# bcgsc/abyss

Measured on AMD Instinct MI355X. Metric: Mk-mers/s inserted+extended (abyss-bloom-dbg, k=64); unitig bit-exact, higher is better.
Workload: dtype u64

## Files before the change

### abyss_amd/_lib.py

```python
from __future__ import annotations

import ctypes as C
import os

from . import build

ABG_OK = 0
ABG_EINVAL, ABG_ENODEV, ABG_ENOMEM, ABG_EINTERNAL, ABG_EAGAIN = -1, -2, -3, -4, -5


class Params(C.Structure):
    _fields_ = [
        ("k", C.c_uint32), ("num_hashes", C.c_uint32), ("min_cov", C.c_uint32), ("trim", C.c_uint32),
        ("bloom_bytes", C.c_uint64), ("counters", C.c_uint64), ("spaced_seed", C.c_char_p),
        ("device", C.c_int32), ("verbose", C.c_int32), ("insert_batch_kmers", C.c_uint64),
        ("claim_log2", C.c_uint32), ("walk_slots", C.c_uint32), ("wtab_log2", C.c_uint32),
        ("cascade_levels", C.c_uint32), ("slice_filter", C.c_uint32), ("reserved_", C.c_uint32 * 5),
    ]


class Counters(C.Structure):
    _fields_ = [(n, C.c_uint64) for n in
                ("solid_reads", "visited_reads", "reads_processed", "bases_assembled", "next_contig_id")]


class Contig(C.Structure):
    _fields_ = [
        ("contig_id", C.c_uint64), ("read_index", C.c_uint64), ("seq", C.c_char_p),
        ("length", C.c_uint32), ("coverage", C.c_uint32), ("redundant", C.c_int32),
        ("left_ext", C.c_uint32), ("right_ext", C.c_uint32), ("left_code", C.c_int32),
        ("right_code", C.c_int32), ("seed_pos", C.c_uint32),
    ]


class Stats(C.Structure):
    _fields_ = [(n, C.c_uint64) for n in
                ("insert_rounds", "walk_rounds", "candidates", "walked", "rewalked", "commit_breaks",
                 "commit_rounds", "generated", "bulk_calls", "bulk_steps", "lin_steps", "guide_slots", "chain_steps", "batch_cuts", "overflows", "memo_hits", "memo_adds", "tiled_ops", "tiled_pending", "tile_overflows", "cls_covered_reads", "archive_bases", "cls_decided_reads", "counter_bytes_held",
                 "commit_rounds_incremental", "commit_dirty_records", "commit_first_chunk_decided")]


CONTIG_CB = C.CFUNCTYPE(None, C.c_void_p, C.POINTER(Contig))
TEXT_CB = C.CFUNCTYPE(None, C.c_void_p, C.POINTER(C.c_char), C.c_uint64)

_lib = None

STAGE_PREFIXES = [("abg_overlap", True), ("abg_rr", True), ("abg_kn", True), ("abg_fm", True), ("abg_de", True), ("abg_ov", True),
                  ("abg_sg", True), ("abg_mc", True), ("abg_pb", False), ("abg_mp", False)]


def symbols():
    return [
        "abg_params_init", "abg_create", "abg_destroy", "abg_last_error", "abg_reset", "abg_filter_size",
        "abg_load_seqs", "abg_load_seqs_v", "abg_keep_reads", "abg_assemble_kept", "abg_load_packed", "abg_counting_stats", "abg_counters_export",
        "abg_counters_import", "abg_visited_export", "abg_visited_import", "abg_assemble_seqs", "abg_assemble_seqs_v",
        "abg_assemble_packed", "abg_cascade_export", "abg_get_counters", "abg_set_counters", "abg_hash_seq",
        "abg_contains_seq",
        "abg_attach_comm", "abg_share_reads", "abg_rccl_unique_id", "abg_rccl_comm_create", "abg_rccl_comm_destroy",
        "abg_dev_copy", "abg_dev_alloc", "abg_dev_free", "abg_output_graph_seqs",
        "abg_profile_enable", "abg_profile_reset", "abg_profile_get", "abg_get_stats",
        "abg_overlap_create", "abg_overlap_destroy", "abg_overlap_last_error", "abg_overlap_join", "abg_overlap_edges",
        "abg_overlap_profile", "abg_overlap_profile_get",
        "abg_rr_create", "abg_rr_destroy", "abg_rr_last_error", "abg_rr_bytes", "abg_rr_clear", "abg_rr_insert_seqs",
        "abg_rr_contains_seqs", "abg_rr_popcount", "abg_rr_export", "abg_rr_sync", "abg_rr_profile", "abg_rr_profile_get",
        "abg_kn_create", "abg_kn_destroy", "abg_kn_last_error", "abg_kn_import", "abg_kn_export", "abg_kn_insert_seqs",
        "abg_kn_contains_seqs", "abg_kn_popcount", "abg_kn_hash_seq", "abg_kn_sync", "abg_kn_profile", "abg_kn_profile_get",
        "abg_fm_create", "abg_fm_destroy", "abg_fm_last_error", "abg_fm_build", "abg_fm_size", "abg_fm_export", "abg_fm_map_seqs",
        "abg_fm_sync", "abg_fm_tune", "abg_fm_profile", "abg_fm_profile_get",
        "abg_de_create", "abg_de_destroy", "abg_de_last_error", "abg_de_set_pmf", "abg_de_scan", "abg_de_estimate", "abg_de_tune",
        "abg_de_profile", "abg_de_profile_get",
        "abg_ov_create", "abg_ov_destroy", "abg_ov_last_error", "abg_ov_set_contigs", "abg_ov_find", "abg_ov_profile",
        "abg_ov_profile_get",
        "abg_sg_create", "abg_sg_destroy", "abg_sg_last_error", "abg_sg_set_graph", "abg_sg_search", "abg_sg_tune", "abg_sg_profile",
        "abg_sg_profile_get",
        "abg_mc_create", "abg_mc_destroy", "abg_mc_last_error", "abg_mc_set_contigs", "abg_mc_merge", "abg_mc_tune", "abg_mc_profile",
        "abg_mc_profile_get",
        "abg_pb_create", "abg_pb_destroy", "abg_pb_last_error", "abg_pb_tune", "abg_pb_align", "abg_pb_align_chain", "abg_pb_profile_get",
        "abg_pb_profile_reset",
        "abg_mp_create", "abg_mp_destroy", "abg_mp_last_error", "abg_mp_tune", "abg_mp_align", "abg_mp_profile_get", "abg_mp_profile_reset",
    ]


def load(path: str | None = None):
    global _lib
    if _lib is not None:
        return _lib
    if path is None:
        path = os.environ.get("ABG_LIB") or build.LIB
        if not os.path.exists(path):
            build.build_lib()
    lib = C.CDLL(path)
    vp, u64p, u8p = C.c_void_p, C.POINTER(C.c_uint64), C.c_void_p
# ... 103 lines not shown
```

### abyss_amd/csrc/abg_engine.h

```cpp
#pragma once
#include "abg_walk.h"

#include <algorithm>
#include <chrono>
#include <cstdio>
#include <cstdlib>
#include <cstring>
#include <functional>
#include <future>
#include <string>
#include <type_traits>
#include <vector>

namespace abg {

struct Failure { int code; std::string msg; };
constexpr int FAIL_INVAL = -1, FAIL_NOMEM = -3, FAIL_INTERNAL = -4;
[[noreturn]] inline void fail_now(int code, const std::string& msg) { throw Failure{ code, msg }; }
inline std::string strf(const char* fmt, unsigned long long a = 0, unsigned long long b = 0)
{
	char buf[256];
	snprintf(buf, sizeof buf, fmt, a, b);
	return buf;
}

struct Config {
	uint32_t k = 0, nh = 4, kc = 2, trim = 0;
	uint64_t counters = 0;
	uint32_t cascade_levels = 0;
	std::string spaced_seed;
	uint64_t insert_batch_kmers = 1ull << 24;
	uint32_t claim_log2 = 30;
	uint32_t drain_threshold = 1u << 12;
	uint64_t compact_threshold = 1u << 20;
	bool async_load = true;
	bool tiled_insert = true;
	bool benign_sharers = true;
	uint32_t cls_debug_skip = 0;
	bool cls_archive = true;
	uint32_t cls_archive_max_mb = 16384;
	bool sorted_overflow = true;
	bool cosettle = true;
	uint32_t cosettle_passes = 6;
	uint32_t cosettle_log2 = 24;
	uint32_t walk_slots = 4096;
	uint32_t tb_cap = 512;
	uint32_t buf_cap = 1u << 16;
	uint64_t pool_cap = 1ull << 28;
	uint32_t rec_cap = 1u << 22;
	uint32_t wtab_log2 = 26;
	uint32_t wtab_log2_max = 31;
	uint32_t cend_log2 = 20;
	uint64_t p2_first_batch = 65536;
	uint64_t p2_max_batch = 1ull << 22;
	uint32_t p2_growth = 2;
	uint32_t p2_crowded = 1u << 18;
	uint32_t p2_starved_growth = 2;
	uint32_t p2_starved = 6144;
	uint32_t slice_filter = 0;
	bool solid_plane = true;
	uint32_t classify_slots = 65536;
	uint32_t cls_both_max_mb = 1024;
	bool cls_both = true;
	bool prefetch_classify = true;
	uint32_t memo_log2 = 0;
	bool memo = true;
	uint32_t p2_max_candidates = 1u << 18;
	uint32_t t_tags = 1024;
	uint32_t commit_incremental = 1;
	uint32_t commit_dirty_max = 4096;
	uint32_t commit_dirty_log2 = 26;
	uint32_t guide_stride = 4;
	uint32_t guide_log2_max = 31;
	bool guide_seen = true;
	bool link_duplicates = true;
	bool par_commit = true;
	bool overlap_bins = true;
	bool overlap_purity = true;
	bool apply_mask = true;
	bool lead_implicit = true;
	uint32_t dist_hash_all_ranks = 2;
	uint32_t dist_route_min_ranks = 4;
	uint64_t keep_insert_scratch_bytes = 16ull << 30;
	uint64_t par_commit_max_bytes = 16ull << 30;
	int verbose = 0;
};

struct Counters {
	uint64_t solid_reads = 0, visited_reads = 0, reads_processed = 0, bases_assembled = 0,
	         contig_id = 0;
};

struct BaseCodes {
	uint8_t t[256];
	BaseCodes()
	{
		for (int i = 0; i < 256; i++) t[i] = 0xFF;
		t['A'] = t['a'] = 0; t['C'] = t['c'] = 1; t['G'] = t['g'] = 2; t['T'] = t['t'] = 3;
	}
};
template <class T>
struct NoInitAlloc : std::allocator<T> {
	template <class U> struct rebind { using other = NoInitAlloc<U>; };
	template <class U, class... A> void construct(U* p, A&&... a)
	{
		if constexpr (sizeof...(A) == 0) ::new ((void*)p) U; else ::new ((void*)p) U(std::forward<A>(a)...);
	}
};
struct HostBatch {
	std::vector<uint32_t, NoInitAlloc<uint32_t>> words;
	std::vector<uint64_t> woff{ 0 };
	std::vector<uint32_t> len;
	std::vector<uint64_t> koff{ 0 };
	void clear() { words.clear(); woff.assign(1, 0); len.clear(); koff.assign(1, 0); }
// ... 2618 lines not shown
						both_set(e.both32, pos);
						if (e.cnt8) { const unsigned c = e.cnt8[pos]; mn = c < mn ? c : mn; }
					}
					if (e.cnt8) cov += mn;
				}
				if (cov) atomic_add_u32(&rec.coverage, cov);
			}
		}
		if (lane == 0) { e.cnt[i] = nrec; e.cnt2[i] = nins; e.cnt3[i] = bases; }
	}
};
struct FPcCover {
	ParCommit e; uint8_t* kmin; uint32_t sum;
	ABG_HDN void operator()(uint64_t i, uint32_t lane, uint32_t nlanes) const
	{
		const uint32_t c = e.c_begin + (uint32_t)i;
		if (c >= e.brk || !e.active[i]) return;
		for (uint32_t ri = e.first_rec[c]; ri != REC_END; ri = e.recs[ri].next) {
			ContigRec& rec = e.recs[ri];
			if (!rec.ins) continue;
			const uint64_t* ch = e.kh + rec.seq_off;
			const uint32_t cnk = rec.len - e.p.k + 1;
			uint32_t cov = 0;
			for (uint32_t j = lane; j < cnk; j += nlanes) {
				if (sum) { cov += kmin[rec.seq_off + j]; continue; }
				const uint64_t h = ch[j];
				unsigned mn = 255;
				for (unsigned q = 0; q < e.p.nh; q++) {
					const uint64_t pos = pos_i(e.p, h, q);
					if (pos - e.own_lo < e.own_span) { const unsigned v = e.cnt8[pos]; mn = v < mn ? v : mn; }
				}
				kmin[rec.seq_off + j] = (uint8_t)mn;
			}
			if (sum && cov) atomic_add_u32(&rec.coverage, cov);
		}
	}
};
struct FPcWrite {
	ParCommit e; uint32_t* order; uint32_t order_base; uint64_t id_base;
	ABG_HD void operator()(uint64_t i, uint32_t) const
	{
		const uint32_t c = e.c_begin + (uint32_t)i;
		if (c >= e.brk || !e.active[i]) return;
		uint32_t o = order_base + e.cnt[i];
		uint64_t id = id_base + e.cnt2[i];
		for (uint32_t ri = e.first_rec[c]; ri != REC_END; ri = e.recs[ri].next) {
			ContigRec& rec = e.recs[ri];
			order[o++] = ri;
			if (rec.ins) rec.contig_id = id++;
		}
	}
};

template <class BE>
class Engine {
  public:
	Engine(BE& be, const Config& cfg) : be_(be), cfg_(cfg)
	{
		uint64_t rem = cfg_.counters % 8;
		m_ = rem ? cfg_.counters + 8 - rem : cfg_.counters;
		p_ = make_params(cfg_.k, cfg_.nh, cfg_.kc, cfg_.trim, m_);
		if (!cfg_.spaced_seed.empty()) {
			MaskTab* mt = new MaskTab;
			make_mask(cfg_.spaced_seed.c_str(), cfg_.k, *mt, p_);
			mask_d_ = (MaskTab*)be_.alloc(sizeof(MaskTab));
			be_.h2d(mask_d_, mt, sizeof(MaskTab));
			delete mt;
			p_.mask = mask_d_;
		}
		if (cfg_.cascade_levels) {
			casc_.levels = cfg_.cascade_levels;
			casc_.level_words = (m_ + 31) / 32;
			casc_.bits = (uint32_t*)be_.alloc(casc_.levels * casc_.level_words * 4);
			be_.memset(casc_.bits, 0, casc_.levels * casc_.level_words * 4);
			cnt_ = (uint8_t*)be_.alloc(8);
			vis_bytes_ = 8;
		} else {
			const uint64_t dev = be_.device_mem_bytes();
			cnt_deferred_ = cfg_.slice_filter == 1 || (cfg_.slice_filter == 0 && dev && (double)m_ * 1.3 > (double)dev * 0.9);
			if (!cnt_deferred_) {
				cnt_ = (uint8_t*)be_.alloc(m_ + 64 * (MAX_RANKS + 1));
				be_.memset(cnt_, 0, m_);
			}
			vis_bytes_ = (m_ / 8 + 4 + 3) & ~3ull;
		}
		vis_ = (uint8_t*)be_.alloc(vis_bytes_);
		be_.memset(vis_, 0, vis_bytes_);
		cstate_ = (CommitState*)be_.alloc(sizeof(CommitState));
		be_.memset(cstate_, 0, sizeof(CommitState));
		scal_ = (uint64_t*)be_.alloc(64);
	}
	~Engine()
	{
		if (BE::ITEM_GROUP_LOG2 == 0 && getenv("ABG_LEAD_COUNT"))
			fprintf(stderr, "lead_stores made=%llu skipped=%llu\n", (unsigned long long)stats_.lead_stores[0], (unsigned long long)stats_.lead_stores[1]);
		free_counters(); be_.free(vis_); if (both_) be_.free(both_); be_.free(cstate_); be_.free(scal_);
		free_archive();
		if (casc_.bits) be_.free(casc_.bits);
		if (mask_d_) be_.free(mask_d_);
		if (T_) be_.free(T_);
		if (Tk_) { be_.free(Tk_); be_.free(Tv_); }
		if (pcA_) be_.free(pcA_);
		if (la_pool_c_) be_.free(la_pool_c_);
		if (la_pool_c2_) be_.free(la_pool_c2_);
		if (guide_tab_) be_.free(guide_tab_);
		if (guide_seen_) be_.free(guide_seen_);
// ... 465 lines not shown
	}
	ContigArchive arc_{}; bool arc_valid_ = false;
	uint64_t loaded_ops_ = 0;
	uint64_t ovf_seen_[2] = { 0, 0 };
	uint8_t* plane_ = nullptr; bool plane_valid_ = false;
	Params p2_; const uint8_t* cnt2_ = nullptr;

	void build_guide(const Batch& b)
	{
		guide_.tab = nullptr; guide_.seen = nullptr; guide_slots_ = 0;
		if (!cfg_.guide_stride || p_.nh > 8 || !b.n) return;
		const uint64_t sampled = (b.n + cfg_.guide_stride - 1) / cfg_.guide_stride;
		uint64_t nwords = 0;
		be_.d2h(&nwords, b.woff + b.n, 8);
		const uint64_t bases = nwords * 16, minus = b.n * (uint64_t)(p_.k - 1);
		const uint64_t kmers = (bases > minus ? bases - minus : b.n) / std::min<uint32_t>(cfg_.guide_stride, 4u);
		uint32_t log2 = 16;
		while ((1ull << log2) < kmers && log2 < cfg_.guide_log2_max) log2++;
		if (!guide_tab_ || log2 != guide_log2_) {
			if (guide_tab_) be_.free(guide_tab_);
			guide_tab_ = (uint64_t*)be_.try_alloc(8ull << log2);
			guide_log2_ = log2;
			if (!guide_tab_) { if (cfg_.verbose) fprintf(stderr, "abyss_amd: no memory for the walkers' guide table, walking step by step\n"); return; }
		}
		be_.memset(guide_tab_, 0, 8ull << log2);
		guide_.mask = (1ull << log2) - 1; guide_.words = b.words; guide_.nwords = nwords;
		dispatch_nw([&](auto nw) {
			FGuideBuild<decltype(nw)::value> f{ p2_, b, cnt2_, guide_tab_, guide_.mask, cfg_.guide_stride, sampled };
			be_.launch_wave((sampled + GUIDE_READS_PER_ITEM - 1) / GUIDE_READS_PER_ITEM, f, "guide_build");
		});
		guide_.tab = guide_tab_;
		guide_slots_ = guide_.mask + 1;
		if (cfg_.guide_seen) {
			const uint64_t need = nwords * 16, total = be_.device_mem_bytes();
			if (guide_seen_ && guide_seen_bytes_ < need) { be_.free(guide_seen_); guide_seen_ = nullptr; }
			if (!guide_seen_ && (!total || need <= total / 24)) { guide_seen_ = (uint8_t*)be_.try_alloc(need); guide_seen_bytes_ = need; }
			if (guide_seen_) { be_.memset(guide_seen_, 0, need); guide_.seen = guide_seen_; }
		}
	}
	uint64_t next_batch_size() const
	{
		if (last_candidates_ > cfg_.p2_crowded) return std::max<uint64_t>(p2_batch_ / 2, 1024);
		if (last_candidates_ < cfg_.p2_starved) return std::min<uint64_t>(p2_batch_ * cfg_.p2_starved_growth, 8 * cfg_.p2_max_batch);
		return std::min<uint64_t>(p2_batch_ * cfg_.p2_growth, cfg_.p2_max_batch);
	}
	void clear_wstats()
	{
		be_.memset(wstats_, 0, WSTAT_N * 8);
	}
	struct Stats { uint64_t rounds = 0, walked = 0, rewalked = 0, candidates = 0, breaks = 0, insert_rounds = 0, commit_rounds = 0, generated = 0;
	               uint64_t bulk_calls = 0, bulk_steps = 0, lin_steps = 0, guide_slots = 0, chain_steps = 0, batch_cuts = 0, overflows = 0, memo_hits = 0, memo_adds = 0;
	               uint64_t tiled_ops = 0, tiled_pending = 0, tile_overflows = 0, cls_covered_reads = 0, archive_bases = 0, cls_decided_reads = 0;
	               uint64_t lead_stores[2] = { 0, 0 };
	               uint64_t commit_rounds_incremental = 0, commit_dirty_records = 0, commit_first_chunk_decided = 0; };
	Stats stats()
	{
		Stats s = stats_;
		if (wstats_) {
			uint64_t v[WSTAT_N];
			be_.d2h(v, wstats_, sizeof v);
			s.bulk_calls = v[WSTAT_BULK_CALLS]; s.bulk_steps = v[WSTAT_BULK_STEPS]; s.lin_steps = v[WSTAT_LIN_STEPS]; s.chain_steps = v[WSTAT_CHAIN_STEPS];
			s.memo_hits = v[WSTAT_MEMO_HITS]; s.memo_adds = v[WSTAT_MEMO_ADDS];
			s.cls_covered_reads = v[WSTAT_CLS_COVERED]; s.cls_decided_reads = v[WSTAT_CLS_DECIDED];
		}
		if (arc_.seq && arc_valid_) { uint64_t u = 0; be_.d2h(&u, arc_.used, 8); s.archive_bases = std::min(u, arc_.cap) - ARC_HEAD; }
		s.guide_slots = guide_slots_;
		return s;
	}

  private:
	BE& be_;
	Config cfg_;
	Params p_;
	uint64_t m_ = 0, vis_bytes_ = 0;
	uint8_t* cnt_ = nullptr;
	uint8_t* vis_ = nullptr;
	CommitState* cstate_ = nullptr;
	uint64_t* scal_ = nullptr;
	Cascade casc_{ nullptr, 0, 0 };
	MaskTab* mask_d_ = nullptr;
	std::chrono::steady_clock::time_point dbg_t0_;
	uint32_t* T_ = nullptr;
	uint32_t t_tag_ = 0;
	uint64_t* Tk_ = nullptr; uint32_t* Tv_ = nullptr; uint32_t Tlog2_ = 0;
	uint64_t T_entries_ = 0;
	uint32_t* pcA_ = nullptr; uint64_t pcA_bits_ = 0; uint32_t pcA_shift_ = 0;
	bool t_hashed() const { return t_force_hashed_ || m_ * 4ull > cfg_.par_commit_max_bytes; }
	bool t_force_hashed_ = false;
	bool use_par_commit()
	{
		if (!cfg_.par_commit || t_failed_) return false;
		if (t_hashed()) return true;
		if (!T_) {
			T_ = (uint32_t*)be_.try_alloc(m_ * 4ull);
			t_tag_ = 0;
			if (!T_ && sliced_) {
				t_force_hashed_ = true;
				if (cfg_.verbose) fprintf(stderr, "abyss_amd: no memory for a time stamp per filter bit, hashed stamps instead\n");
				return true;
			}
			if (!T_) { t_failed_ = true; if (cfg_.verbose) fprintf(stderr, "abyss_amd: no memory for the parallel commit's time stamps, using the ordered kernel\n"); return false; }
		}
		return true;
	}
	bool t_failed_ = false;
	Comm comm_;
	bool force_dist_ = false, comm_scaled_ = false;
	bool sliced_ = false, cnt_deferred_ = false; uint64_t win_total_ = 0, win_span_ = 0, win_lo_ = 0;
	bool cnt_loaded_ = false;
	uint64_t own_lo_ = 0, own_span_ = 0, own_chunk_ = 0;
	uint8_t* tred_ = nullptr;
	bool cnt_partial_ = false;
	uint32_t* sh_words_ = nullptr; uint64_t* sh_woff_ = nullptr; uint32_t* sh_len_ = nullptr; uint64_t* sh_koff_ = nullptr;
	uint8_t* dres_ = nullptr; uint8_t* dlost_ = nullptr;
	TilePair* rsend_ = nullptr; TilePair* rrecv_ = nullptr; uint32_t rcap_ = 0; uint64_t rrecv_cap_ = 0; uint32_t* rslot_ = nullptr; uint32_t* rcur_ = nullptr;
	uint8_t* rrep_out_ = nullptr; uint8_t* rrep_in_ = nullptr; uint8_t* rtgt_out_ = nullptr; uint8_t* rtgt_in_ = nullptr; uint8_t* rpendf_ = nullptr;
	uint64_t rown_ = 0;
	bool routed() const
	{
// ... 627 lines not shown
			be_.launch(npend, f, "route_pend");
			if (big) { be_.sync(); be_.free(big); }
			FClaimOwned fc{ p_, h0_, pend_[1], claim_[0], cmask, epoch_, own_lo_, own_span_ };
			be_.launch(npend, fc, "claim_list");
		}
		insert_rounds_dist(T, cmask, pend_[1], npend);
	}
	void insert_rounds_dist(uint64_t T, uint64_t cmask, const uint32_t* pin, uint64_t npend)
	{
		(void)T;
		cnt_partial_ = true;
		uint64_t* ccur = claim_[0];
		uint64_t* cnext = claim_[1];
		uint32_t* pout = pend_[0];
		while (npend) {
			if (pin && npend <= cfg_.drain_threshold) {
				uint8_t* val = dres_;
				{ FDrainVals f{ p_, h0_, cnt_, pin, own_lo_, own_span_, val }; be_.launch(npend, f, "drain_vals"); }
				c_all_reduce(val, npend * p_.nh, DT_U8, OP_MAX);
				{ FDrainLoad f{ p_, h0_, cnt_, pin, own_lo_, own_span_, val, ccur, cmask, epoch_ }; be_.launch(npend, f, "drain_load"); }
				uint32_t* other = (pin == pend_[0]) ? pend_[1] : pend_[0];
				InsertDrainEnv de{ p_, h0_, cnt_, casc_, const_cast<uint32_t*>(pin), other, (uint32_t)npend,
					ccur, cnext, cmask, epoch_, pend_n_ };
				be_.launch_drain(de);
				uint32_t r[2] = { 0, 0 };
				be_.d2h(r, pend_n_, 8);
				epoch_ += r[1];
				last_rounds_ += r[1];
				stats_.insert_rounds += r[1];
				break;
			}
			{ FEvalDist f{ p_, h0_, cnt_, pin, ccur, cmask, epoch_, own_lo_, own_span_, dres_ }; be_.launch(npend, f, pin ? "insert_retry" : "insert_round"); }
			c_all_reduce(dres_, npend, DT_U8, OP_MIN);
			{ FApplyDist f{ p_, h0_, cnt_, pin, cnext, cmask, epoch_, own_lo_, own_span_, dres_, dlost_ }; be_.launch(npend, f, "insert_apply"); }
			be_.compact_flagged(pin, dlost_, npend, pout, pend_n_);
			uint32_t nn = 0;
			be_.d2h(&nn, pend_n_, 4);
			npend = nn;
			std::swap(ccur, cnext);
			pin = pout;
			pout = (pout == pend_[0]) ? pend_[1] : pend_[0];
			epoch_++;
			last_rounds_++;
			stats_.insert_rounds++;
		}
		epoch_++;
	}

	void ensure_walk()
	{
		if (walk_ready_) return;
		if (!cend_.hmin) {
			p2_batch_ = cfg_.p2_first_batch;
			cslots_ = std::min<uint32_t>(be_.max_slots(), cfg_.classify_slots);
			alloc_tab(cend_, cfg_.cend_log2);
		}
		wslots_ = std::min<uint32_t>(be_.max_slots(), cfg_.walk_slots);
		wtab_log2_ = cfg_.wtab_log2;
		alloc_tab(wtab_, wtab_log2_);
		la_pool_ = (VKey*)be_.alloc((uint64_t)wslots_ * LA_MAX_VISITED * sizeof(VKey));
		bulk_pool_ = (BulkScratch*)be_.alloc((uint64_t)wslots_ * sizeof(BulkScratch));
		if (!wstats_) { wstats_ = (uint64_t*)be_.alloc(WSTAT_N * 8); clear_wstats(); }
		walk_tb_cap_ = cfg_.tb_cap;
		walk_buf_cap_ = cfg_.buf_cap;
		alloc_walk_scratch();
		pool_cap_ = cfg_.pool_cap;
		pool_ = (uint8_t*)be_.alloc(pool_cap_);
		kh_ = (uint64_t*)be_.alloc(pool_cap_ * 8);
		pool_used_ = (uint64_t*)be_.alloc(8);
		rec_cap_ = cfg_.rec_cap;
		recs_ = (ContigRec*)be_.alloc((uint64_t)rec_cap_ * sizeof(ContigRec));
		rec_used_ = (uint32_t*)be_.alloc(8);
		order_ = (uint32_t*)be_.alloc((uint64_t)rec_cap_ * 4);
		order_n_ = (uint32_t*)be_.alloc(8);
		walk_ready_ = true;
	}
	void alloc_walk_scratch()
	{
		tb_pool_ = be_.alloc((uint64_t)wslots_ * walk_tb_cap_ * sizeof(TBFrame<NW_MASKED + MAX_NW>));
		tbk_pool_ = (VKey*)be_.alloc((uint64_t)wslots_ * walk_tb_cap_ * sizeof(VKey));
		lbuf_ = (uint8_t*)be_.alloc((uint64_t)wslots_ * walk_buf_cap_);
		rbuf_ = (uint8_t*)be_.alloc((uint64_t)wslots_ * walk_buf_cap_);
	}
	void free_walk_scratch() { be_.free(tb_pool_); be_.free(tbk_pool_); be_.free(lbuf_); be_.free(rbuf_); }
	void alloc_tab(WalkTab& t, uint32_t log2)
	{
		uint64_t cap = 1ull << log2;
		t.hmin = (uint64_t*)be_.alloc(cap * 8);
		t.hmax = (uint64_t*)be_.alloc(cap * 8);
		t.meta = (uint64_t*)be_.alloc(cap * 8);
		t.mask = cap - 1;
		be_.memset(t.hmin, 0xFF, cap * 8);
		be_.memset(t.meta, 0xFF, cap * 8);
	}
	void free_tab(WalkTab& t) { be_.free(t.hmin); be_.free(t.hmax); be_.free(t.meta); }
	void free_walk()
	{
		if (!walk_ready_) return;
		free_tab(wtab_);
		be_.free(la_pool_); be_.free(bulk_pool_);
		free_walk_scratch();
		be_.free(pool_); be_.free(kh_); be_.free(pool_used_); be_.free(recs_); be_.free(rec_used_);
		be_.free(order_); be_.free(order_n_);
		walk_ready_ = false;
	}
	void grow_walk_resources()
	{
// ... 431 lines not shown
		uint32_t* need_d = nullptr; uint32_t* need_n = nullptr; uint64_t* rkoff_d = nullptr;
		uint32_t base = 0;
		uint32_t prepped = 0, owner_next = 0, committed = 0, force = 0xFFFFFFFFu, nneed = 0, nneed_all = 0;
		bool round_started = false;
		bool predicted = false;
		bool pending = false;
		bool overflow = false, debug = false;
	};
	template <int NW>
	void assemble_nw(const Batch& b, uint8_t* result_d, uint8_t* results_host,
	    const std::function<void(const ContigOut&)>& sink)
	{
		uint64_t next = 0;
		while (next < b.n) {
			ensure_walk();
			BatchRun r;
			classify_batch<NW>(b, next, std::min<uint64_t>(p2_batch_, b.n - next), result_d, r);
			next += r.n;
			counters_.reads_processed += r.n;
			p2_batch_ = next_batch_size();
			prefetch_ = nullptr;
			if (next < b.n && !dist() && cfg_.prefetch_classify) {
				const uint64_t nf = next, nn = std::min<uint64_t>(p2_batch_, b.n - next);
				prefetch_ = [this, &b, result_d, nf, nn]() {
					if (!la_pool_c2_) la_pool_c2_ = (VKey*)be_.alloc((uint64_t)cslots_ * LA_MAX_VISITED * sizeof(VKey));
					Batch vn = b;
					vn.woff = b.woff + nf; vn.len = b.len + nf; vn.koff = b.koff + nf; vn.n = nn;
					FClassify<NW> f{ p2_, vn, 0, cnt2_, vis_, result_d + nf, la_pool_c2_, both_, arc_, cfg_.cls_debug_skip };
					be_.launch_slots_side(nn, f, cslots_, "classify");
					pre_first_ = nf; pre_n_ = nn;
				};
			}
			if (r.nc) {
				setup_batch<NW>(r);
				finish_batch<NW>(r, sink);
			}
			if (results_host) {
				be_.d2h(results_host + r.first, r.res_d, r.n);
				if (const void* left = memchr(results_host + r.first, RES_CANDIDATE, r.n)) {
					fail_now(FAIL_INTERNAL, strf("read %llu left unprocessed", (unsigned long long)((const uint8_t*)left - results_host)));
				}
			}
		}
	}

	template <int NW>
	void classify_batch(const Batch& b, uint64_t first, uint64_t n, uint8_t* result_d, BatchRun& r)
	{
		Batch v = b;
		v.woff = b.woff + first; v.len = b.len + first; v.koff = b.koff + first; v.n = n;
		uint8_t* res_d = result_d + first;
		if (!la_pool_c_) la_pool_c_ = (VKey*)be_.alloc((uint64_t)cslots_ * LA_MAX_VISITED * sizeof(VKey));
		if (pre_n_ == n && pre_first_ == first) {
			be_.sync_side();
			FRefilter<NW> f{ p_, v, vis_, res_d };
			be_.launch(n, f, "reclassify");
		} else if (dist()) {
			const uint64_t R = (uint64_t)comm_.world;
			std::vector<uint64_t> c(R), d(R);
			for (uint64_t q = 0; q < R; q++) { d[q] = n * q / R; c[q] = n * (q + 1) / R - d[q]; }
			FClassify<NW> f{ p2_, v, d[comm_.rank], cnt2_, vis_, res_d, la_pool_c_ };
			be_.launch_slots(c[comm_.rank], f, cslots_, "classify");
			c_all_gather_v(res_d, c.data(), d.data());
		} else {
			be_.sync_side();
			FClassify<NW> f{ p2_, v, 0, cnt2_, vis_, res_d, la_pool_c_, both_, arc_, cfg_.cls_debug_skip };
			be_.launch_slots(n, f, cslots_, "classify");
		}
		pre_n_ = 0;
		std::vector<uint8_t> res(n);
		be_.d2h(res.data(), res_d, n);
		r = BatchRun();
		uint64_t used = n;
		const uint64_t max_cand = std::min<uint64_t>(cfg_.p2_max_candidates,
		    std::max<uint64_t>(1024, (1ull << wtab_log2_cap()) / (2 * wtab_per_walker_)));
		for (const uint8_t* q = res.data(), *end = q + n; (q = (const uint8_t*)memchr(q, RES_CANDIDATE, (size_t)(end - q))) != nullptr; q++) {
			if (r.cand_h.size() >= max_cand) { used = (uint64_t)(q - res.data()); break; }
			r.cand_h.push_back((uint32_t)(q - res.data()));
		}
		uint64_t n_visited = 0;
		for (uint64_t i = 0; i < used; i++) n_visited += res[i] == RR_ALL_KMERS_VISITED;
		counters_.solid_reads += n_visited + r.cand_h.size();
		counters_.visited_reads += n_visited;
		v.n = used;
		r.v = v; r.first = first; r.n = used; r.res_d = res_d;
		r.nc = (uint32_t)r.cand_h.size();
		if (used < n) stats_.batch_cuts++;
		stats_.candidates += r.nc;
		last_candidates_ = r.nc;
	}

	template <int NW>
	void setup_batch(BatchRun& r)
	{
		const uint32_t nc = r.nc;
		const Batch& b = r.v;
		r.cand_d = (uint32_t*)be_.alloc(nc * 4ull);
		r.status_d = (uint32_t*)be_.alloc(nc * 4ull);
		r.first_d = (uint32_t*)be_.alloc(nc * 4ull);
		r.need_d = (uint32_t*)be_.alloc(nc * 4ull);
		r.need_n = (uint32_t*)be_.alloc(8);
		be_.h2d(r.cand_d, r.cand_h.data(), nc * 4ull);
		std::vector<uint32_t> len_h(nc);
		{
			uint32_t* cl = (uint32_t*)be_.alloc(nc * 4ull + 4);
			FGatherU32 f{ b.len, r.cand_d, cl };
			be_.launch(nc, f, "gather_len");
// ... 221 lines not shown
```

### abyss_amd/csrc/abg_kernels.hip

```cpp
#include <hip/hip_runtime.h>
#include <hip/hip_ext.h>
#include <hipcub/hipcub.hpp>
#include <rccl/rccl.h>
#include <dlfcn.h>
#include <unistd.h>

#include "abg_host.h"
#include "abg_overlap.h"

#include <chrono>
#include <map>
#include <mutex>

namespace {

template <class F>
__global__ void __launch_bounds__(256) k_foreach(F f, uint64_t n)
{
	uint64_t i = (uint64_t)blockIdx.x * blockDim.x + threadIdx.x;
	const uint64_t stride = (uint64_t)gridDim.x * blockDim.x;
	const uint32_t slot = (uint32_t)i;
	for (; i < n; i += stride) f(i, slot);
}
#ifndef ABG_CLS_WAVES
#define ABG_CLS_WAVES 3
#endif
template <class F>
__global__ void __launch_bounds__(64, ABG_CLS_WAVES) k_foreach_w(F f, uint64_t n)
{
	uint64_t i = (uint64_t)blockIdx.x * blockDim.x + threadIdx.x;
	const uint64_t stride = (uint64_t)gridDim.x * blockDim.x;
	const uint32_t slot = (uint32_t)i;
	for (; i < n; i += stride) f(i, slot);
}

#ifndef ABG_WALK_WAVES
#define ABG_WALK_WAVES 3
#endif
#ifndef ABG_WALK_LDS
#define ABG_WALK_LDS 13312
#endif
constexpr uint32_t WALK_LDS = ABG_WALK_LDS;
template <class F>
__global__ void __launch_bounds__(64, ABG_WALK_WAVES) k_walkers(F f, uint64_t n, unsigned long long* ticket)
{
	__shared__ __attribute__((aligned(16))) unsigned char lds[WALK_LDS];
	{
		abg::MaskCache* mc = (abg::MaskCache*)(lds + WALK_LDS - sizeof(abg::MaskCache));
		for (unsigned i = threadIdx.x; i < abg::MC_N; i += 64) mc->valid[i] = 0;
		__builtin_amdgcn_fence(__ATOMIC_ACQ_REL, "wavefront");
	}
	for (;;) {
		unsigned long long i = 0;
		if (threadIdx.x == 0) i = atomicAdd(ticket, 1ull);
		i = ((unsigned long long)(unsigned)__builtin_amdgcn_readfirstlane((int)(i >> 32)) << 32) |
		    (unsigned)__builtin_amdgcn_readfirstlane((int)(unsigned)i);
		if (i >= n) break;
		f(i, (uint32_t)blockIdx.x, (void*)lds, WALK_LDS, true);
	}
}

template <class F>
__global__ void __launch_bounds__(256) k_foreach_wave(F f, uint64_t n)
{
	const uint32_t lane = threadIdx.x & 63;
	uint64_t w = ((uint64_t)blockIdx.x * blockDim.x + threadIdx.x) >> 6;
	const uint64_t nw = ((uint64_t)gridDim.x * blockDim.x) >> 6;
	for (; w < n; w += nw) f(w, lane, 64u);
}

constexpr int COMMIT_THREADS = 256;
constexpr int SYNC_WORDS = 34;
struct DeviceSync {
	uint32_t* sh;
	abg::CommitDesc* dsc = nullptr;
	__device__ abg::CommitDesc* descs() { return dsc; }
	__device__ uint32_t tid() const { return threadIdx.x; }
	__device__ uint32_t nthreads() const { return blockDim.x; }
	__device__ void barrier() { __syncthreads(); }
	__device__ bool all(bool v) { return __syncthreads_and(v ? 1 : 0) != 0; }
	__device__ uint32_t sum(uint32_t v)
	{
		for (int o = 32; o > 0; o >>= 1) v += __shfl_down(v, o, 64);
		__syncthreads();
		if ((threadIdx.x & 63) == 0) sh[threadIdx.x >> 6] = v;
		__syncthreads();
// ... 36 lines not shown
{
	__shared__ uint32_t sh[SYNC_WORDS];
	__shared__ abg::CommitDesc dsc[abg::COMMIT_CHUNK];
	DeviceSync sy{ sh, dsc };
	abg::commit_candidates<NW>(e, c_begin, c_end, sy);
}

template <class F>
__global__ void __launch_bounds__(F::THREADS) k_tiles(F f, uint64_t n)
{
	__shared__ __attribute__((aligned(16))) unsigned char lds[F::FAST];
	DeviceSync sy{ nullptr };
	for (uint64_t tile = blockIdx.x; tile < n; tile += gridDim.x) {
		f(tile, (void*)lds, sy);
		__syncthreads();
	}
}

__global__ void __launch_bounds__(1024) k_insert_drain(abg::InsertDrainEnv e)
{
	__shared__ uint32_t sh[SYNC_WORDS];
	DeviceSync sy{ sh };
	abg::insert_drain(e, sy);
}

struct ProfEntry { double ms = 0; uint64_t launches = 0; };

struct HipBackend {
	static constexpr uint32_t ITEM_GROUP_LOG2 = 6;
	int device = 0;
	bool good = false;
	std::string reason;
	hipStream_t stream = nullptr;
	hipStream_t stream2 = nullptr;
	hipEvent_t ev2a = nullptr, ev2b = nullptr;
	std::string side_name;
	bool side_pending = false;
	bool profiling = false;
	std::map<std::string, ProfEntry> prof;
	uint32_t cus = 256;
	unsigned long long* ticket = nullptr;

	explicit HipBackend(int dev = 0) : device(dev)
	{
		int n = 0;
		hipError_t e = hipGetDeviceCount(&n);
		if (e != hipSuccess || n <= 0) { reason = "no HIP device available (abyss_amd has no CPU fallback)"; return; }
		if (dev < 0 || dev >= n) { reason = "HIP device ordinal out of range"; return; }
		if (hipSetDevice(dev) != hipSuccess) { reason = "hipSetDevice failed"; return; }
		hipDeviceProp_t prop;
		if (hipGetDeviceProperties(&prop, dev) == hipSuccess) cus = (uint32_t)prop.multiProcessorCount;
		if (hipStreamCreate(&stream) != hipSuccess) { reason = "hipStreamCreate failed"; return; }
		if (const char* e = getenv("ABG_MEM_LIMIT_MB")) mem_limit = (size_t)strtoull(e, 0, 10) << 20;
		{
			int lo = 0, hi = 0;
			hipDeviceGetStreamPriorityRange(&lo, &hi);
			const char* e = getenv("ABG_SIDE_PRIORITY");
			const bool low = !e || atoi(e) != 0;
			if (hipStreamCreateWithPriority(&stream2, hipStreamNonBlocking, low ? lo : hi) != hipSuccess) { reason = "hipStreamCreate failed"; return; }
		}
		hipEventCreate(&ev2a);
		hipEventCreate(&ev2b);
		good = true;
	}
	~HipBackend()
	{
		if (ticket) free(ticket);
		if (pin) hipHostFree(pin);
		for (int i = 0; i < 2; i++) { if (big_pin[i]) hipHostFree(big_pin[i]); if (big_ev[i]) hipEventDestroy(big_ev[i]); }
		for (int i = 0; i < 2; i++) { if (ahead_pin[i]) hipHostFree(ahead_pin[i]); if (ahead_ev[i]) hipEventDestroy(ahead_ev[i]); if (ahead[i].dev) hipFree(ahead[i].dev); }
		for (void* q : ahead_old) hipFree(q);
		if (ahead_stream) hipStreamDestroy(ahead_stream);
		if (cub_tmp) hipFree(cub_tmp);
		drop_cache();
		prof_drain(true);
		for (auto& q : prof_free) { hipEventDestroy(q.first); hipEventDestroy(q.second); }
		if (ev2a) hipEventDestroy(ev2a);
		if (ev2b) hipEventDestroy(ev2b);
		if (stream2) hipStreamDestroy(stream2);
		if (stream) hipStreamDestroy(stream);
	}
	bool ok() const { return good; }
	std::string why() const { return reason; }
	void bind_thread() { (void)hipSetDevice(device); }
	static void check(hipError_t e, const char* what)
	{
		if (e != hipSuccess) {
			(void)hipGetLastError();
			abg::fail_now(e == hipErrorOutOfMemory ? abg::FAIL_NOMEM : abg::FAIL_INTERNAL, std::string(what) + " failed: " + hipGetErrorString(e));
		}
	}
	static constexpr size_t CACHE_MAX_BLOCK = 256ull << 20, CACHE_MAX_TOTAL = 8ull << 30;
	std::map<size_t, std::vector<void*>> cache_free;
	std::map<void*, size_t> cache_size;
	size_t cache_held = 0;
	size_t mem_limit = 0, mem_used = 0;
	std::map<void*, size_t> mem_size;
	hipError_t dev_malloc(void** p, size_t n)
	{
		if (mem_limit && mem_used + n > mem_limit) return hipErrorOutOfMemory;
		const hipError_t e = hipMalloc(p, n);
		if (e == hipSuccess && mem_limit) { mem_used += n; mem_size[*p] = n; }
		return e;
	}
	void dev_free(void* p)
	{
		if (mem_limit) { auto it = mem_size.find(p); if (it != mem_size.end()) { mem_used -= it->second; mem_size.erase(it); } }
		hipFree(p);
	}
	void* try_alloc(size_t n)
	{
		void* p = nullptr;
		hipSetDevice(device);
		if (dev_malloc(&p, n ? n : 1) != hipSuccess) { (void)hipGetLastError(); return nullptr; }
		if (getenv("ABG_MEM_DEBUG")) fprintf(stderr, "[mem] +%.2f GB (optional)\n", n / 1e9);
		return p;
	}
	void* alloc(size_t n)
	{
		void* p = nullptr;
// ... 243 lines not shown
		hipEventRecord(prof_cur.first, stream);
	}
	void end(const char* name)
	{
		check(hipGetLastError(), name);
		if (!profiling || !prof_cur.first) return;
		hipEventRecord(prof_cur.second, stream);
		prof_pending.push_back({ prof_cur.first, prof_cur.second, &prof[name] });
		prof_cur = { nullptr, nullptr };
		if (prof_pending.size() >= 8192) prof_drain();
	}
	void prof_drain(bool discard = false)
	{
		for (ProfPending& q : prof_pending) {
			if (!discard && hipEventSynchronize(q.b) == hipSuccess) {
				float ms = 0;
				if (hipEventElapsedTime(&ms, q.a, q.b) == hipSuccess) { q.p->ms += ms; q.p->launches++; }
			}
			prof_free.push_back({ q.a, q.b });
		}
		prof_pending.clear();
	}
	template <class K, class... A>
	void launch_kernel(const char* name, K kernel, dim3 grid, dim3 block, A... args)
	{
		if (!profiling) {
			hipLaunchKernelGGL(kernel, grid, block, 0, stream, args...);
			check(hipGetLastError(), name);
			return;
		}
		if (prof_free.empty()) { hipEvent_t a, b; hipEventCreate(&a); hipEventCreate(&b); prof_free.push_back({ a, b }); }
		const std::pair<hipEvent_t, hipEvent_t> ev = prof_free.back(); prof_free.pop_back();
		hipExtLaunchKernelGGL(kernel, grid, block, 0, stream, ev.first, ev.second, 0, args...);
		check(hipGetLastError(), name);
		prof_pending.push_back({ ev.first, ev.second, &prof[name] });
		if (prof_pending.size() >= 8192) prof_drain();
	}
	template <class F>
	void launch(uint64_t n, F f, const char* name)
	{
		if (!n) return;
		uint64_t blocks = (n + 255) / 256;
		uint64_t cap = (uint64_t)cus * 8;
		if (blocks > cap) blocks = cap;
		launch_kernel(name, k_foreach<F>, dim3((uint32_t)blocks), dim3(256), f, n);
	}
	template <class F>
	void launch_slots(uint64_t n, F f, uint32_t slots, const char* name)
	{
		if (!n) return;
		uint64_t blocks = (n + 63) / 64;
		uint64_t cap = slots / 64 ? slots / 64 : 1;
		if (blocks > cap) blocks = cap;
		launch_kernel(name, k_foreach_w<F>, dim3((uint32_t)blocks), dim3(64), f, n);
	}
	template <class F>
	void launch_slots_side(uint64_t n, F f, uint32_t slots, const char* name)
	{
		if (!n) return;
		uint64_t blocks = (n + 63) / 64;
		uint64_t cap = slots / 64 ? slots / 64 : 1;
		if (blocks > cap) blocks = cap;
		hipEventRecord(ev2a, stream);
		hipStreamWaitEvent(stream2, ev2a, 0);
		hipEventRecord(ev2a, stream2);
		hipLaunchKernelGGL(k_foreach_w<F>, dim3((uint32_t)blocks), dim3(64), 0, stream2, f, n);
		check(hipGetLastError(), name);
		hipEventRecord(ev2b, stream2);
		side_name = name;
		side_pending = true;
	}
	hipEvent_t evs0 = nullptr, evs1 = nullptr;
	bool scope_pending = false, scope_saved_prof = false;
	std::string scope_name;
	void side_scope_begin(const char* name)
	{
		if (!evs0) { hipEventCreate(&evs0); hipEventCreate(&evs1); }
		scope_name = name;
		hipEventRecord(evs0, stream);
		hipStreamWaitEvent(stream2, evs0, 0);
		std::swap(stream, stream2);
		scope_saved_prof = profiling; profiling = false;
		hipEventRecord(evs0, stream);
	}
	void side_scope_end()
	{
		hipEventRecord(evs1, stream);
		std::swap(stream, stream2);
		profiling = scope_saved_prof;
		scope_pending = true;
	}
	void wait_side_scope()
	{
		if (!scope_pending) return;
		check(hipEventSynchronize(evs1), "hipEventSynchronize");
		if (profiling) {
			float ms = 0;
			hipEventElapsedTime(&ms, evs0, evs1);
			ProfEntry& p = prof[scope_name];
			p.ms += ms;
			p.launches++;
		}
		scope_pending = false;
	}
	bool side_done() { return !side_pending || hipEventQuery(ev2b) == hipSuccess; }
	void sync_side()
	{
		if (!side_pending) return;
		check(hipEventSynchronize(ev2b), "hipEventSynchronize");
		if (profiling) {
			float ms = 0;
			hipEventElapsedTime(&ms, ev2a, ev2b);
			ProfEntry& p = prof[side_name];
			p.ms += ms;
			p.launches++;
		}
		side_pending = false;
	}
	template <class F>
// ... 474 lines not shown
		return ctx->s.output_graph_seqs(seqs, offsets, n, cb, user, nodes, edges);
	});
}
int abg_profile_enable(abg_ctx* ctx, int on)
{
	if (!ctx) return ABG_EINVAL;
	return guarded(ctx, [&]() -> int {
		ctx->s.be.prof_drain();
		ctx->s.be.profiling = on != 0;
		return ABG_OK;
	});
}
int abg_profile_reset(abg_ctx* ctx)
{
	if (!ctx) return ABG_EINVAL;
	return guarded(ctx, [&]() -> int {
		ctx->s.be.prof_drain(true);
		ctx->s.be.prof.clear();
		return ABG_OK;
	});
}
int abg_profile_get(abg_ctx* ctx, const char* name, double* total_ms, uint64_t* launches)
{
	if (!ctx || !name) return ABG_EINVAL;
	return guarded(ctx, [&]() -> int {
		ctx->s.be.prof_drain();
		auto it = ctx->s.be.prof.find(name);
		double ms = 0;
		uint64_t n = 0;
		if (it != ctx->s.be.prof.end()) { ms = it->second.ms; n = it->second.launches; }
		if (total_ms) *total_ms = ms;
		if (launches) *launches = n;
		return ABG_OK;
	});
}
int abg_get_stats(const abg_ctx* ctx, abg_stats* out)
{
	if (!ctx || !out) return ABG_EINVAL;
	return guarded((abg_ctx*)ctx, [&]() -> int {
		auto s = ctx->s.eng->stats();
		out->insert_rounds = s.insert_rounds;
		out->walk_rounds = s.rounds;
		out->candidates = s.candidates;
		out->walked = s.walked;
		out->rewalked = s.rewalked;
		out->commit_breaks = s.breaks; out->commit_rounds = s.commit_rounds; out->generated = s.generated;
		out->bulk_calls = s.bulk_calls; out->bulk_steps = s.bulk_steps; out->lin_steps = s.lin_steps; out->guide_slots = s.guide_slots; out->chain_steps = s.chain_steps; out->batch_cuts = s.batch_cuts; out->overflows = s.overflows;
		out->memo_hits = s.memo_hits; out->memo_adds = s.memo_adds;
		out->tiled_ops = s.tiled_ops; out->tiled_pending = s.tiled_pending; out->tile_overflows = s.tile_overflows;
		out->cls_covered_reads = s.cls_covered_reads; out->archive_bases = s.archive_bases; out->cls_decided_reads = s.cls_decided_reads;
		out->counter_bytes_held = ctx->s.eng->counter_bytes_held();
		out->commit_rounds_incremental = s.commit_rounds_incremental; out->commit_dirty_records = s.commit_dirty_records;
		out->commit_first_chunk_decided = s.commit_first_chunk_decided;
		return ABG_OK;
	});
}

}
struct abg_overlap {
	HipBackend be;
	abg::OverlapJoin<HipBackend> join;
	std::string error;
	explicit abg_overlap(int dev) : be(dev), join(be) {}
};
namespace {
std::string g_overlap_create_error;
template <class F>
int guarded_ov(abg_overlap* o, F&& body)
{
	try {
		return body();
	} catch (const abg::Failure& f) {
		o->error = f.msg;
		return f.code;
	} catch (const std::bad_alloc&) {
		o->error = "host memory exhausted";
		return ABG_ENOMEM;
	} catch (const std::exception& e) {
		o->error = e.what();
		return ABG_EINTERNAL;
	}
}
}
extern "C" {
int abg_overlap_create(int device, abg_overlap** out)
{
	if (!out) return ABG_EINVAL;
	*out = nullptr;
	abg_overlap* o = nullptr;
	try {
		o = new abg_overlap(device);
	} catch (const std::exception& e) {
		g_overlap_create_error = e.what();
		return ABG_EINTERNAL;
	}
	if (!o->be.ok()) {
		g_overlap_create_error = o->be.why();
		delete o;
		return ABG_ENODEV;
	}
	*out = o;
	return ABG_OK;
}
void abg_overlap_destroy(abg_overlap* o) { delete o; }
const char* abg_overlap_last_error(const abg_overlap* o) { return o ? o->error.c_str() : g_overlap_create_error.c_str(); }
int abg_overlap_join(abg_overlap* o, uint32_t overlap, uint64_t n_contigs, const uint64_t* head_keys, const uint64_t* tail_keys,
// ... 38 lines not shown
```

### include/abyss_amd.h

```cpp
#ifndef ABYSS_AMD_H
#define ABYSS_AMD_H 1

#include <stddef.h>
#include <stdint.h>

#ifdef __cplusplus
extern "C" {
#endif

#define ABG_OK 0
#define ABG_EINVAL (-1)
#define ABG_ENODEV (-2)
#define ABG_ENOMEM (-3)
#define ABG_EINTERNAL (-4)
#define ABG_EAGAIN (-5)

#define ABG_MAX_KMER 192
#define ABG_MAX_HASHES 32

enum abg_read_result {
	ABG_RR_UNINITIALIZED = 0,
	ABG_RR_SHORTER_THAN_K,
	ABG_RR_NON_ACGT,
	ABG_RR_BLUNT_END,
// ... 100 lines not shown
	int32_t rank, world;
	int32_t stream_ordered;
	int32_t struct_size;
	void* user;
	int (*all_gather_v)(void* user, void* buf, const uint64_t* counts, const uint64_t* displs, void* stream);
	int (*all_reduce)(void* user, void* buf, uint64_t count, int32_t dtype, int32_t op, void* stream);
	int (*all_to_all_v)(void* user, const void* send, const uint64_t* send_counts, const uint64_t* send_displs,
	    void* recv, const uint64_t* recv_counts, const uint64_t* recv_displs, void* stream);
} abg_comm;
#define ABG_MAX_RANKS 16

int abg_attach_comm(abg_ctx* ctx, const abg_comm* comm);

int abg_share_reads(abg_ctx* ctx, const uint32_t* d_words, const uint64_t* d_woff, const uint32_t* d_len,
    uint64_t n_local, const uint32_t** g_words, const uint64_t** g_woff, const uint32_t** g_len,
    uint64_t* n_total);

int abg_rccl_unique_id(uint8_t id[128]);
int abg_rccl_comm_create(const uint8_t id[128], int32_t rank, int32_t world, int32_t device, abg_comm* out);
int abg_rccl_comm_destroy(abg_comm* comm);

int abg_dev_copy(abg_ctx* ctx, void* dst, const void* src, uint64_t n, int32_t kind);
int abg_dev_alloc(abg_ctx* ctx, uint64_t bytes, void** out);
int abg_dev_free(abg_ctx* ctx, void* ptr);

typedef void (*abg_text_cb)(void* user, const char* text, uint64_t len);
int abg_output_graph_seqs(abg_ctx* ctx, const char* seqs, const uint64_t* offsets, uint64_t n,
    abg_text_cb cb, void* user, uint64_t* nodes, uint64_t* edges);

int abg_profile_enable(abg_ctx* ctx, int on);
int abg_profile_reset(abg_ctx* ctx);
int abg_profile_get(abg_ctx* ctx, const char* name, double* total_ms, uint64_t* launches);
typedef struct abg_stats {
	uint64_t insert_rounds, walk_rounds, candidates, walked, rewalked, commit_breaks;
	uint64_t commit_rounds;
	uint64_t generated;
	uint64_t bulk_calls, bulk_steps;
	uint64_t lin_steps;
	uint64_t guide_slots;
	uint64_t chain_steps;
	uint64_t batch_cuts;
	uint64_t overflows;
	uint64_t memo_hits, memo_adds;
	uint64_t tiled_ops;
	uint64_t tiled_pending;
	uint64_t tile_overflows;
	uint64_t cls_covered_reads;
	uint64_t archive_bases;
	uint64_t cls_decided_reads;
	uint64_t counter_bytes_held;
	uint64_t commit_rounds_incremental;
	uint64_t commit_dirty_records;
	uint64_t commit_first_chunk_decided;
} abg_stats;
int abg_get_stats(const abg_ctx* ctx, abg_stats* out);

typedef struct abg_overlap abg_overlap;
int abg_overlap_create(int device, abg_overlap** out);
void abg_overlap_destroy(abg_overlap* o);
const char* abg_overlap_last_error(const abg_overlap* o);
int abg_overlap_join(abg_overlap* o, uint32_t overlap, uint64_t n_contigs, const uint64_t* head_keys,
    const uint64_t* tail_keys, int strand_specific, uint64_t* n_edges);
int abg_overlap_edges(abg_overlap* o, uint64_t* offsets, uint32_t* targets);
int abg_overlap_profile(abg_overlap* o, int on);
int abg_overlap_profile_get(abg_overlap* o, const char* name, double* total_ms, uint64_t* launches);

typedef struct abg_rr abg_rr;
int abg_rr_create(int device, uint64_t bytes, uint32_t hash_num, uint32_t r, abg_rr** out);
void abg_rr_destroy(abg_rr* f);
const char* abg_rr_last_error(const abg_rr* f);
int abg_rr_bytes(const abg_rr* f, uint64_t* bytes);
int abg_rr_clear(abg_rr* f);
int abg_rr_insert_seqs(abg_rr* f, const char* seqs, const uint64_t* offsets, uint64_t n, uint32_t max_bases,
    const uint32_t* lengths, uint32_t n_lengths, uint64_t* n_inserted);
int abg_rr_contains_seqs(abg_rr* f, const char* seqs, const uint64_t* offsets, uint64_t n, uint32_t* found);
int abg_rr_popcount(abg_rr* f, uint64_t* bits_set);
int abg_rr_export(abg_rr* f, uint8_t* host_out);
int abg_rr_sync(abg_rr* f);
int abg_rr_profile(abg_rr* f, int on);
int abg_rr_profile_get(abg_rr* f, const char* name, double* total_ms, uint64_t* launches);


typedef struct abg_kn abg_kn;
int abg_kn_create(int device, uint64_t full_bits, uint32_t levels, uint32_t k, uint64_t seed, uint64_t start, uint64_t end,
    abg_kn** out);
void abg_kn_destroy(abg_kn* f);
const char* abg_kn_last_error(const abg_kn* f);
int abg_kn_import(abg_kn* f, uint32_t level, const uint8_t* bytes);
int abg_kn_export(abg_kn* f, uint32_t level, uint8_t* bytes);
int abg_kn_insert_seqs(abg_kn* f, const char* seqs, const uint64_t* offsets, uint64_t n);
int abg_kn_contains_seqs(abg_kn* f, const char* seqs, const uint64_t* offsets, uint64_t n, int inverse, uint8_t* print);
int abg_kn_popcount(abg_kn* f, uint64_t* per_level);
int abg_kn_hash_seq(abg_kn* f, const char* seq, uint64_t len, uint64_t* hash, uint64_t* index, uint8_t* valid);
int abg_kn_sync(abg_kn* f);
int abg_kn_profile(abg_kn* f, int on);
int abg_kn_profile_get(abg_kn* f, const char* name, double* total_ms, uint64_t* launches);

typedef struct abg_fm abg_fm;
typedef struct abg_fm_hit { uint32_t l, u, qstart, qend, num, pos; } abg_fm_hit;
#define ABG_FM_NO_RC 1u
#define ABG_FM_SS 2u
int abg_fm_create(int device, abg_fm** out);
void abg_fm_destroy(abg_fm* f);
const char* abg_fm_last_error(const abg_fm* f);
int abg_fm_build(abg_fm* f, const uint8_t* text, uint64_t n);
int abg_fm_size(const abg_fm* f, uint64_t* n);
// ... 96 lines not shown
```

Before: 1714.

## Size classify lanes to device occupancy and balance classify work with atomic tickets

The classify lane count now defaults to the device's resident wave capacity (CUs × 4 × waves × 64) instead of a fixed 65536. It falls back to the small size when the doubled look-ahead pools would use more than an eighth of free device memory. Classify kernels, on both the main and side streams, now use a persistent-wave loop where each wave claims 64-element chunks through an atomic ticket counter, rather than a fixed grid stride. This targets load imbalance across uneven per-read look-ahead work, at the cost of larger pools, an extra memset per launch, and one atomic per chunk. Side-stream wait time and lane count are also exposed as stats.

```diff
diff --git a/abyss_amd/_lib.py b/abyss_amd/_lib.py
--- a/abyss_amd/_lib.py
+++ b/abyss_amd/_lib.py
@@ -37,7 +37,7 @@
     _fields_ = [(n, C.c_uint64) for n in
                 ("insert_rounds", "walk_rounds", "candidates", "walked", "rewalked", "commit_breaks",
                  "commit_rounds", "generated", "bulk_calls", "bulk_steps", "lin_steps", "guide_slots", "chain_steps", "batch_cuts", "overflows", "memo_hits", "memo_adds", "tiled_ops", "tiled_pending", "tile_overflows", "cls_covered_reads", "archive_bases", "cls_decided_reads", "counter_bytes_held",
-                 "commit_rounds_incremental", "commit_dirty_records", "commit_first_chunk_decided")]
+                 "commit_rounds_incremental", "commit_dirty_records", "commit_first_chunk_decided")] + [("cls_wait_ms", C.c_double), ("cls_lanes", C.c_uint64)]
 
 
 CONTIG_CB = C.CFUNCTYPE(None, C.c_void_p, C.POINTER(Contig))
diff --git a/abyss_amd/csrc/abg_engine.h b/abyss_amd/csrc/abg_engine.h
--- a/abyss_amd/csrc/abg_engine.h
+++ b/abyss_amd/csrc/abg_engine.h
@@ -59,7 +59,7 @@
 	uint32_t p2_starved = 6144;
 	uint32_t slice_filter = 0;
 	bool solid_plane = true;
-	uint32_t classify_slots = 65536;
+	uint32_t classify_slots = 0;
 	uint32_t cls_both_max_mb = 1024;
 	bool cls_both = true;
 	bool prefetch_classify = true;
@@ -2784,6 +2784,11 @@
 	}
 };
 
+constexpr uint32_t CLS_SLOTS_SMALL = 65536;
+template <class BE> auto classify_lanes(BE& be, int) -> decltype(be.classify_lanes()) { return be.classify_lanes(); }
+template <class BE> uint32_t classify_lanes(BE&, long) { return CLS_SLOTS_SMALL; }
+template <class BE> auto device_mem_free(BE& be, int) -> decltype(be.device_mem_free()) { return be.device_mem_free(); }
+template <class BE> uint64_t device_mem_free(BE&, long) { return 0; }
 template <class BE>
 class Engine {
   public:
@@ -3355,7 +3360,9 @@
 	               uint64_t bulk_calls = 0, bulk_steps = 0, lin_steps = 0, guide_slots = 0, chain_steps = 0, batch_cuts = 0, overflows = 0, memo_hits = 0, memo_adds = 0;
 	               uint64_t tiled_ops = 0, tiled_pending = 0, tile_overflows = 0, cls_covered_reads = 0, archive_bases = 0, cls_decided_reads = 0;
 	               uint64_t lead_stores[2] = { 0, 0 };
-	               uint64_t commit_rounds_incremental = 0, commit_dirty_records = 0, commit_first_chunk_decided = 0; };
+	               uint64_t commit_rounds_incremental = 0, commit_dirty_records = 0, commit_first_chunk_decided = 0;
+	               double cls_wait_ms = 0;
+	               uint64_t cls_lanes = 0; };
 	Stats stats()
 	{
 		Stats s = stats_;
@@ -3368,6 +3375,7 @@
 		}
 		if (arc_.seq && arc_valid_) { uint64_t u = 0; be_.d2h(&u, arc_.used, 8); s.archive_bases = std::min(u, arc_.cap) - ARC_HEAD; }
 		s.guide_slots = guide_slots_;
+		s.cls_lanes = cslots_;
 		return s;
 	}
 
@@ -4101,7 +4109,11 @@
 		if (walk_ready_) return;
 		if (!cend_.hmin) {
 			p2_batch_ = cfg_.p2_first_batch;
-			cslots_ = std::min<uint32_t>(be_.max_slots(), cfg_.classify_slots);
+			cslots_ = std::min<uint32_t>(be_.max_slots(), cfg_.classify_slots ? cfg_.classify_slots : classify_lanes(be_, 0));
+			if (!cfg_.classify_slots && cslots_ > CLS_SLOTS_SMALL) {
+				const uint64_t pools = 2ull * cslots_ * LA_MAX_VISITED * sizeof(VKey), free_now = device_mem_free(be_, 0);
+				if (pools > free_now / 8) cslots_ = CLS_SLOTS_SMALL;
+			}
 			alloc_tab(cend_, cfg_.cend_log2);
 		}
 		wslots_ = std::min<uint32_t>(be_.max_slots(), cfg_.walk_slots);
@@ -4639,7 +4651,9 @@
 		uint8_t* res_d = result_d + first;
 		if (!la_pool_c_) la_pool_c_ = (VKey*)be_.alloc((uint64_t)cslots_ * LA_MAX_VISITED * sizeof(VKey));
 		if (pre_n_ == n && pre_first_ == first) {
+			const auto t_wait = std::chrono::steady_clock::now();
 			be_.sync_side();
+			stats_.cls_wait_ms += std::chrono::duration<double, std::milli>(std::chrono::steady_clock::now() - t_wait).count();
 			FRefilter<NW> f{ p_, v, vis_, res_d };
 			be_.launch(n, f, "reclassify");
 		} else if (dist()) {
diff --git a/abyss_amd/csrc/abg_kernels.hip b/abyss_amd/csrc/abg_kernels.hip
--- a/abyss_amd/csrc/abg_kernels.hip
+++ b/abyss_amd/csrc/abg_kernels.hip
@@ -32,6 +32,20 @@
 	const uint64_t stride = (uint64_t)gridDim.x * blockDim.x;
 	const uint32_t slot = (uint32_t)i;
 	for (; i < n; i += stride) f(i, slot);
+}
+template <class F>
+__global__ void __launch_bounds__(64, ABG_CLS_WAVES) k_foreach_wt(F f, uint64_t n, unsigned long long* ticket)
+{
+	const uint32_t slot = blockIdx.x * 64u + threadIdx.x;
+	for (;;) {
+		unsigned long long t = 0;
+		if (threadIdx.x == 0) t = atomicAdd(ticket, 1ull);
+		t = ((unsigned long long)(unsigned)__builtin_amdgcn_readfirstlane((int)(t >> 32)) << 32) |
+		    (unsigned)__builtin_amdgcn_readfirstlane((int)(unsigned)t);
+		if (t * 64 >= n) break;
+		const uint64_t i = t * 64 + threadIdx.x;
+		if (i < n) f(i, slot);
+	}
 }
 
 #ifndef ABG_WALK_WAVES
@@ -174,6 +188,7 @@
 		if (hipGetDeviceProperties(&prop, dev) == hipSuccess) cus = (uint32_t)prop.multiProcessorCount;
 		if (hipStreamCreate(&stream) != hipSuccess) { reason = "hipStreamCreate failed"; return; }
 		if (const char* e = getenv("ABG_MEM_LIMIT_MB")) mem_limit = (size_t)strtoull(e, 0, 10) << 20;
+		if (const char* e = getenv("ABG_CLS_TICKETS")) cls_tickets = atoi(e) != 0;
 		{
 			int lo = 0, hi = 0;
 			hipDeviceGetStreamPriorityRange(&lo, &hi);
@@ -188,6 +203,7 @@
 	~HipBackend()
 	{
 		if (ticket) free(ticket);
+		if (cls_ticket_) free(cls_ticket_);
 		if (pin) hipHostFree(pin);
 		for (int i = 0; i < 2; i++) { if (big_pin[i]) hipHostFree(big_pin[i]); if (big_ev[i]) hipEventDestroy(big_ev[i]); }
 		for (int i = 0; i < 2; i++) { if (ahead_pin[i]) hipHostFree(ahead_pin[i]); if (ahead_ev[i]) hipEventDestroy(ahead_ev[i]); if (ahead[i].dev) hipFree(ahead[i].dev); }
@@ -537,7 +553,25 @@
 		uint64_t blocks = (n + 63) / 64;
 		uint64_t cap = slots / 64 ? slots / 64 : 1;
 		if (blocks > cap) blocks = cap;
-		launch_kernel(name, k_foreach_w<F>, dim3((uint32_t)blocks), dim3(64), f, n);
+		if (!cls_tickets) { launch_kernel(name, k_foreach_w<F>, dim3((uint32_t)blocks), dim3(64), f, n); return; }
+		unsigned long long* t = cls_ticket(0);
+		check(hipMemsetAsync(t, 0, 8, stream), "hipMemsetAsync");
+		launch_kernel(name, k_foreach_wt<F>, dim3((uint32_t)blocks), dim3(64), f, n, t);
+	}
+	bool cls_tickets = true;
+	unsigned long long* cls_ticket_ = nullptr;
+	unsigned long long* cls_ticket(int side)
+	{
+		if (!cls_ticket_) cls_ticket_ = (unsigned long long*)alloc(256);
+		return cls_ticket_ + (side ? 16 : 0);
+	}
+	uint32_t classify_lanes() const { return cus * 4 * ABG_CLS_WAVES * 64; }
+	uint64_t device_mem_free() const
+	{
+		size_t fr = 0, tot = 0;
+		if (hipMemGetInfo(&fr, &tot) != hipSuccess) { (void)hipGetLastError(); return 0; }
+		if (mem_limit) fr = std::min(fr, mem_limit > mem_used ? mem_limit - mem_used : (size_t)0);
+		return fr;
 	}
 	template <class F>
 	void launch_slots_side(uint64_t n, F f, uint32_t slots, const char* name)
@@ -548,8 +582,11 @@
 		if (blocks > cap) blocks = cap;
 		hipEventRecord(ev2a, stream);
 		hipStreamWaitEvent(stream2, ev2a, 0);
+		unsigned long long* t = cls_tickets ? cls_ticket(1) : nullptr;
+		if (t) check(hipMemsetAsync(t, 0, 8, stream2), "hipMemsetAsync");
 		hipEventRecord(ev2a, stream2);
-		hipLaunchKernelGGL(k_foreach_w<F>, dim3((uint32_t)blocks), dim3(64), 0, stream2, f, n);
+		if (t) hipLaunchKernelGGL(k_foreach_wt<F>, dim3((uint32_t)blocks), dim3(64), 0, stream2, f, n, t);
+		else hipLaunchKernelGGL(k_foreach_w<F>, dim3((uint32_t)blocks), dim3(64), 0, stream2, f, n);
 		check(hipGetLastError(), name);
 		hipEventRecord(ev2b, stream2);
 		side_name = name;
@@ -1130,6 +1167,7 @@
 		out->counter_bytes_held = ctx->s.eng->counter_bytes_held();
 		out->commit_rounds_incremental = s.commit_rounds_incremental; out->commit_dirty_records = s.commit_dirty_records;
 		out->commit_first_chunk_decided = s.commit_first_chunk_decided;
+		out->cls_wait_ms = s.cls_wait_ms; out->cls_lanes = s.cls_lanes;
 		return ABG_OK;
 	});
 }
diff --git a/include/abyss_amd.h b/include/abyss_amd.h
--- a/include/abyss_amd.h
+++ b/include/abyss_amd.h
@@ -176,6 +176,8 @@
 	uint64_t commit_rounds_incremental;
 	uint64_t commit_dirty_records;
 	uint64_t commit_first_chunk_decided;
+	double cls_wait_ms;
+	uint64_t cls_lanes;
 } abg_stats;
 int abg_get_stats(const abg_ctx* ctx, abg_stats* out);
 
```

Result: faster. 1760 (median of 6 runs) (+2.7%).
